# Deltares/pyflwdir

Hardware: AMD Instinct MI355X
Metric: Mcells/s upstream_area on D8 raster (higher is better)
Workload: dtype int32

## Files before the change

### pyflwdir_amd/csrc/tiled.h

```cpp
#pragma once
#include "common.h"

#define TS 64
#define TCELLS (TS * TS)
#define HW (TS + 2)
#define PSL 256
#define SG 8
#define SSL (SG * SG * PSL)
#define SSHIFT 14
#define SDONE 0x8000u
#define MAXROUNDS_SUPER 15
#define HG 4
#define HCAP 24576
#define HDONE 0x8000u
#define NPERIM (2 * TS + 2 * (TS - 2))
#define NONE32 0xFFFFFFFFu
#define PDONE 0x8000u
#define XDONE 0x80000000u
#define MAXROUNDS_TILE 13
#define CPT (TCELLS / 256)
#define ENC_SINK 0x80000000u
#define ENC_SIDE1 0x40000000u
#define ENC_COL 0x3FFFFFFFu

// ... 19 lines not shown
}
__host__ __device__ inline u32 xr_target12(u32 tr, u32 tc, u32 t12, u32 nstc);

__host__ __device__ inline u32 xr_target12(u32 tr, u32 tc, u32 t12, u32 nstc) {
  const u32 d = t12 >> 8;
  const u32 q = (d * 11u) >> 5;
  return sslot_base(tr + q - 1u, tc + (d - 3u * q) - 1u, nstc) + (t12 & 0xFFu);
}

__host__ __device__ inline u32 sb_index(u32 R, u32 C) {
  return R == 0u ? C : (R == SC - 1u ? SC + C : (C == 0u ? 2u * SC + (R - 1u) : 2u * SC + (SC - 2u) + (R - 1u)));
}
__host__ __device__ inline void sb_cell(u32 t, u32 *R, u32 *C) {
  if (t < SC) *R = 0u, *C = t;
  else if (t < 2u * SC) *R = SC - 1u, *C = t - SC;
  else if (t < 2u * SC + (SC - 2u)) *R = t - 2u * SC + 1u, *C = 0u;
  else *R = (t - (2u * SC + (SC - 2u)) + 1u) & (SC - 1u), *C = SC - 1u;
}

struct SuperArgs {
  u32 nst;
  const u32 *xT;
  const u32 *xrec;
  const u64 *xmask;
  uint16_t *xcb;
  uint16_t *xl_slot;
  uint16_t *xl_next;
  u32 *scount;
  u32 *nflag, *flagged;
  u32 *sb;
  uint16_t *R2L;
  u32 *sxidL;
  u32 *sx_slot;
  u32 *sx_n1;
  u32 *T3;
  u32 *xtot;
  u64 *ctrl;
  u32 nstc, nhtc;
  u32 *hcnt;
  int hmode;
  u32 edge_nstr;
  u32 ntr, ntc;
  u32 hcap;
  u8 *sover;
  u32 scap;
};

struct HyperArgs {
  const u32 *sx_slot;
  u32 *xtot;
  u32 nht;
  const u32 *hcnt;
  const u32 *T3;
  const u32 *J3;
  const u32 *xin3;
  u32 *T3out;
  u32 *R3;
  u32 *hx_id;
  u32 *hx_node;
  u32 *T4;
  u64 *ctrl;
  u32 edge_nstr, nhtc;
};

struct TileArgs {
  const u8 *ncode;
  const u8 *raw;
  u8 *ncode_w;
  u64 *tcnt;
  u64 ntot;
  u32 *hcnt;
  u32 nht;
  const i32 *weights;
  u32 nrow, ncol, ntr, ntc;
  u32 row_first, row_last;
  u32 nstc;
  u32 *xT;
  u32 *xrec;
  const u32 *xtot;
  u64 *xmask;
  u32 *esink;
  u32 *brow_first;
  u32 *haloA;
  u32 *brow_inflow;
  u64 *ctrl;
  i32 *out;
  u32 tr_lo, tr_hi, tc_lo, tc_hi;
  u64 *rcnt;
  u64 *stamps;
  int flags;
  const u64 *wrow = nullptr;
  const u32 *wfrac = nullptr;
  u64 *xT64 = nullptr;
};

__host__ __device__ inline u32 frame_tiles(u32 ntr, u32 ntc, u32 tr_lo, u32 tr_hi, u32 tc_lo, u32 tc_hi) {
  return ntr * ntc - (tr_hi - tr_lo) * (tc_hi - tc_lo);
}
__host__ __device__ inline void frame_tile(u32 id, u32 ntr, u32 ntc, u32 tr_lo, u32 tr_hi, u32 tc_lo, u32 tc_hi, u32 *tr,
                                           u32 *tc) {
  const u32 top = tr_lo * ntc, bot = (ntr - tr_hi) * ntc;
  if (id < top) {
    *tr = id / ntc, *tc = id % ntc;
  } else if (id < top + bot) {
    id -= top;
    *tr = tr_hi + id / ntc, *tc = id % ntc;
  } else {
    id -= top + bot;
    const u32 side = tc_lo + (ntc - tc_hi);
    const u32 x = id % side;
    *tr = tr_lo + id / side;
    *tc = x < tc_lo ? x : tc_hi + (x - tc_lo);
  }
}

// ... 65 lines not shown
    const i64 crr = gr < 0 ? 0 : (gr >= (i64)nrow ? (i64)nrow - 1 : gr);
    const i64 ccs = cs < 0 ? 0 : (cs >= (i64)ncol ? (i64)ncol - 1 : cs);
    u32 w;
    size_t off = (size_t)crr * ncol + (size_t)ccs;
    u32 sh = 0;
    if (GUARD && off + 4 > ntot) {
      sh = 8u * (u32)(off + 4 - ntot);
      off = ntot - 4;
    }
    __builtin_memcpy(&w, ncode + off, 4);
    if (GUARD) w >>= sh;
    const bool rowok = idx < HW * 18u && gr >= 0 && gr < (i64)nrow;
#pragma unroll
    for (int b = 0; b < 4; ++b) {
      const i64 col = cs + b;
      if (!rowok || col < 0 || col >= (i64)ncol) w = (w & ~(0xFFu << (8 * b))) | (D8_MV << (8 * b));
    }
    v[k] = w;
  }
}
__device__ __forceinline__ void stage_load_interior(const u8 *__restrict__ ncode, u32 ncol, i64 r0, i64 c0, u32 tid,
                                                    u32 (&v)[5]) {
  const u8 *base = ncode + (size_t)(r0 - 1) * ncol + (size_t)(c0 - 4);
#pragma unroll
  for (int k = 0; k < 5; ++k) {
    const u32 idx = tid + 256u * k;
    u32 hr = idx / 18u;
    const u32 d = idx - hr * 18u;
    hr = hr < HW - 1u ? hr : HW - 1u;
    __builtin_memcpy(&v[k], base + (size_t)hr * ncol + 4u * d, 4);
  }
}
__device__ __forceinline__ void stage_load_auto(const u8 *__restrict__ ncode, u32 nrow, u32 ncol, i64 r0, i64 c0, u32 tid,
                                                u32 (&v)[5]) {
  if (r0 >= 1 && c0 >= 4 && r0 + TS + 1 <= (i64)nrow && c0 + TS + 4 <= (i64)ncol) stage_load_interior(ncode, ncol, r0, c0, tid, v);
  else stage_load(ncode, nrow, ncol, r0, c0, tid, v);
}
__device__ __forceinline__ void stage_store(u8 *code, u32 tid, const u32 (&v)[5]) {
#pragma unroll
  for (int k = 0; k < 5; ++k) {
    const u32 idx = tid + 256u * k;
    if (idx < HW * 18u) ((u32 *)code)[idx] = v[k];
  }
}
#endif

struct TiledRun {
  pfd_raster *h = nullptr;
  u32 ntr = 0, ntc = 0, nexits = 0;
  size_t nslots = 0;
  bool supported = false, is_block = false, coarse_done = false, force_flat = false;
  DevBuf slots, sx, esink, bnd;
  u32 nst = 0, nstc = 0, nsuper = 0, nht = 0, nhtc = 0, nhyper = 0;
  DevBuf sbbuf, l3, l4, hcntbuf, tcntbuf, iface_buf, stampbuf, soverbuf, rcntbuf, xmaskbuf, xlbuf, scountbuf, flaggedbuf, xcbbuf;
  bool fused_norm = false;
  int rounds4 = 0, extra_rounds = 0;
  bool short_of_rounds = false;
  u32 *xT = nullptr, *xrec = nullptr, *xtot = nullptr, *sxidL = nullptr, *sx_slot = nullptr,
      *sx_n1 = nullptr;
  uint16_t *R2L = nullptr;
  SuperArgs sa{};
  u32 *brow_first = nullptr, *haloA = nullptr, *haloL = nullptr, *brow_sink = nullptr, *brow_inflow = nullptr;
  u32 *Tc = nullptr, *Tn = nullptr, *Jc = nullptr, *Jn = nullptr, *xin3 = nullptr, *R3 = nullptr, *hx_id = nullptr;
  size_t n3cap = 0, n4cap = 0;
  u32 *J4fin = nullptr;
  int solve_exits(const u32 *start, i64 *launches, bool cleared = false, bool edge_down = false);
  bool edge_down_now = false;
  int level3_flat(i64 *launches);
  int level3_flat_nosync(i64 *launches);
  bool flat_nosync = false;
  int level3_hyper(i64 *launches);
  int level4_down(i64 *launches);
  int resolve_with_inflow(i64 *launches);
  TileArgs a{};
  int init(pfd_raster *hh, i32 *out_dev);
  bool overflowed = false;
  int phase_a();
  int phase_a_checked();
  int phase_a_check();
  int phase_b(int *complete);
  int phase_b_issue();
  int phase_b_collect(const u64 *c0, int *complete);
  int stage_verdict_a();
  int block_verdict(int *flag_dev, bool host_ok);
  bool iface_doubling = false;
  u64 last_miss = 0;
  bool phase_a_needs_redo(const u64 *c8, int tries);
};

int pfd_doubling_rounds(pfd_raster *h, u32 *T[3], u32 *J[2], u32 n, int first_batch, bool check, bool *done,
                        int *rounds_issued, i64 *launches, const u64 *ncnt = nullptr, bool prepared = false);
```

### pyflwdir_amd/csrc/tiled.hip

```cpp
#include <stdio.h>
#include <stdlib.h>

#include <vector>

#include "common.h"
#include "tiled.h"

#define TSTAMP(slot)                                                                                        \
  if (a.flags & 16) {                                                                                       \
    __syncthreads();                                                                                        \
    if (tid == 0) {                                                                                         \
      const u64 t_ = __builtin_readcyclecounter();                                                          \
      atomicAdd((unsigned long long *)&a.stamps[(((tr * a.ntc + tc) & 1023u) << 3) + (FINAL ? 4 : 0) + slot], \
                (unsigned long long)(t_ - tprev));                                                        \
      tprev = t_;                                                                                           \
    }                                                                                                       \
  }

#define PREP 8
template <bool FINAL, bool RAW, bool INT, bool PERIM>
__device__ __forceinline__ void tile_body(const TileArgs &a, u32 *A, uint16_t *P, u8 *code, u64 *s_cnt, const u32 tr,
                                          const u32 tc) {
  u64 tprev = __builtin_readcyclecounter();
  const u32 tid = threadIdx.x;
// ... 686 lines not shown
      tot += c;
    }
    if (!tot) {
      s_base = 0;
    } else if (s.hmode) {
      const u32 b = atomicAdd(&s.hcnt[ht], tot);
      if (b + tot > s.hcap) s.ctrl[T_OVERFLOW] = 1;
      s_base = ht * HCAP + (b + tot > s.hcap ? 0u : b);
    } else {
      s_base = (u32)atomicAdd((unsigned long long *)&s.ctrl[T_NSUPER], (unsigned long long)tot);
    }
  }
  __syncthreads();
  u32 run = s_base + wtot[wave];
#pragma unroll
  for (int k = 0; k < DPT; ++k) {
    const u32 e = tid + NT * k;
    const bool sx = (sxbits >> k) & 1u;
    const u64 m = __ballot(sx);
    u32 id = NONE32;
    if (sx) {
      id = run + (u32)__popcll(m & ((1ull << lane) - 1ull));
      const u32 sl = (u32)s.xl_slot[base + e] & (SSL - 1);
      s.sx_slot[id] = base + sl;
      s.sx_n1[id] = xr_target12(str * SG + (sl >> 11), stc * SG + ((sl >> 8) & 7u), (u32)s.xl_next[base + e] & 0xFFFu, s.nstc);
      s.T3[id] = T[e];
    }
    run += (u32)__popcll(m);
    if (e < n) {
      s.R2L[base + e] = (uint16_t)(P[e] & (SDONE - 1u));
      s.sxidL[base + e] = id;
    }
  }
}

template <bool FINAL>
__global__ void __launch_bounds__(SNT, SNT == 512u ? 6 : 8) k_super(SuperArgs s) {
  if (s.sover[blockIdx.x]) return;
  super_solve<FINAL, SCAP, SNT>(s, blockIdx.x);
}
#define SFLAG_GRID 64u
template <bool FINAL>
__global__ void __launch_bounds__(1024, 4) k_super_flagged(SuperArgs s) {
  const u32 nf = *s.nflag;
  for (u32 f = blockIdx.x; f < nf; f += gridDim.x) {
    super_solve<FINAL, SSL, 1024u>(s, s.flagged[f]);
    __syncthreads();
  }
}

__device__ __forceinline__ bool sx_active(const SuperArgs &s, u32 k) {
  return !s.hmode || (k % HCAP) < s.hcnt[k / HCAP];
}
__global__ void __launch_bounds__(256) k_link3(SuperArgs s, u32 nsuper, u32 *__restrict__ J3,
                                               u32 *__restrict__ clear = nullptr) {
  const u32 k = blockIdx.x * blockDim.x + threadIdx.x;
  if (k >= nsuper) return;
  if (clear) clear[k] = 0;
  if (s.hmode && s.ctrl[T_OVERFLOW]) return;
  if (!sx_active(s, k)) {
    J3[k] = k | XDONE;
    return;
  }
  const u32 tgt = s.sx_n1[k];
  const u32 xe = (s.xrec[tgt] >> 8) & 0xFFu;
  u32 j = k | XDONE, pos = NONE32;
  if (xe != XR_NONE) {
    const u32 n1 = (tgt & ~255u) | xe, b1 = n1 & ~(u32)(SSL - 1);
    pos = b1 + xl_index(s.xmask, s.xcb, n1);
    const u32 id = s.sxidL[b1 + s.R2L[pos]];
    if (id != NONE32) j = id;
  }
  s.sx_n1[k] = pos;
  J3[k] = j;
}
__global__ void __launch_bounds__(256) k_sx_totals(SuperArgs s, u32 nsuper, const u32 *__restrict__ T3final) {
  const u32 k = blockIdx.x * blockDim.x + threadIdx.x;
  if (k < nsuper) s.xtot[s.sx_slot[k]] = T3final[k];
}

__global__ void __launch_bounds__(256) k_link3_flat(SuperArgs s, u32 cap, u32 *__restrict__ J3, u32 *__restrict__ Tnext) {
  const u32 n = min(cap, (u32)s.ctrl[T_NSUPER]);
  for (u32 k = blockIdx.x * blockDim.x + threadIdx.x; k < n; k += gridDim.x * blockDim.x) {
    Tnext[k] = 0;
    const u32 tgt = s.sx_n1[k];
    const u32 xe = (s.xrec[tgt] >> 8) & 0xFFu;
    u32 j = k | XDONE, pos = NONE32;
    if (xe != XR_NONE) {
      const u32 n1 = (tgt & ~255u) | xe, b1 = n1 & ~(u32)(SSL - 1);
      pos = b1 + xl_index(s.xmask, s.xcb, n1);
      const u32 id = s.sxidL[b1 + s.R2L[pos]];
      if (id != NONE32) j = id;
    }
    s.sx_n1[k] = pos;
    J3[k] = j;
  }
}
__global__ void __launch_bounds__(256) k_sx_totals_flat(SuperArgs s, u32 cap, const u32 *__restrict__ T3final) {
  const u32 n = min(cap, (u32)s.ctrl[T_NSUPER]);
  for (u32 k = blockIdx.x * blockDim.x + threadIdx.x; k < n; k += gridDim.x * blockDim.x) s.xtot[s.sx_slot[k]] = T3final[k];
}

template <bool FINAL>
__global__ void __launch_bounds__(1024) k_hyper(HyperArgs s) {
  __shared__ u32 T[HCAP];
  __shared__ uint16_t P[HCAP];
  __shared__ __attribute__((aligned(16))) u32 s_flag[2][16];
  __shared__ u32 s_cnt, s_base;
  const u32 tid = threadIdx.x;
  const u32 ht = blockIdx.x;
  const u32 base = ht * HCAP;
  if (s.ctrl[T_OVERFLOW]) return;
  if (FINAL && s.edge_nstr) {
    const u32 hr = ht / s.nhtc, n_ = s.edge_nstr;
    if (hr != 0 && hr < (n_ >= 3 ? (n_ - 3) / HG : 0u)) return;
  }
  const u32 n = s.hcnt[ht];
  constexpr int SPT = HCAP / 1024;
  if (tid == 0) s_cnt = 0;
  u32 y[SPT], ext = 0, live = 0;
#pragma unroll
  for (int j0 = 0; j0 < SPT; j0 += 8) {
    u32 j3s[8], ts[8];
    if (1024u * j0 < n) {
#pragma unroll
      for (int q = 0; q < 8; ++q) {
        const u32 i = tid + 1024u * (j0 + q);
        j3s[q] = s.J3[base + i];
        ts[q] = s.T3[base + i];
        if (FINAL) ts[q] += s.xin3[base + i];
      }
    }
#pragma unroll
    for (int q = 0; q < 8; ++q) {
      const int j = j0 + q;
      const u32 i = tid + 1024u * j;
      u32 p = i | HDONE, t = 0;
      if (i < n) {
        const u32 j3 = j3s[q];
        t = ts[q];
        if (!(j3 & XDONE)) {
          if (j3 / HCAP == ht)
            p = j3 % HCAP;
          else
            ext |= 1u << j;
        }
      }
      T[i] = t;
      P[i] = (uint16_t)p;
      y[j] = p & 0x7FFFu;
      if (!(p & HDONE)) live |= 1u << j;
    }
  }
  __syncthreads();
  for (int round = 0; round < 16; ++round) {
    u32 av[SPT], q[SPT];
#pragma unroll
    for (int j = 0; j < SPT; ++j) {
      if (live & (1u << j)) {
        av[j] = T[tid + 1024u * j];
        q[j] = P[y[j]];
      }
    }
    __syncthreads();
#pragma unroll
    for (int j = 0; j < SPT; ++j) {
      if (live & (1u << j)) {
        atomicAdd(&T[y[j]], av[j]);
        P[tid + 1024u * j] = (uint16_t)q[j];
        y[j] = q[j] & 0x7FFFu;
        if (q[j] & HDONE) live &= ~(1u << j);
      }
    }
    if (!wg_vote<16>(s_flag, round, tid, live != 0u)) break;
  }
  if (live) atomicAdd((unsigned long long *)&s.ctrl[T_SLIVE], 1ull);
  if (FINAL) {
#pragma unroll
    for (int j = 0; j < SPT; ++j) {
      const u32 i = tid + 1024u * j;
      if (i < n) {
        s.T3out[base + i] = T[i];
        s.xtot[s.sx_slot[base + i]] = T[i];
      }
    }
    return;
  }
  u32 rank[SPT];
#pragma unroll
  for (int j = 0; j < SPT; ++j) rank[j] = (ext & (1u << j)) ? atomicAdd(&s_cnt, 1u) : NONE32;
  __syncthreads();
  if (tid == 0) s_base = s_cnt ? (u32)atomicAdd((unsigned long long *)&s.ctrl[T_NHYPER], (unsigned long long)s_cnt) : 0u;
  __syncthreads();
#pragma unroll
  for (int j = 0; j < SPT; ++j) {
    const u32 i = tid + 1024u * j;
    if (i >= n) continue;
    s.T3out[base + i] = T[i];
    s.R3[base + i] = base + (P[i] & 0x7FFFu);
    u32 id = NONE32;
    if (rank[j] != NONE32) {
      id = s_base + rank[j];
      s.hx_node[id] = base + i;
      s.T4[id] = T[i];
    }
    s.hx_id[base + i] = id;
  }
}
__global__ void __launch_bounds__(256) k_link4(HyperArgs s, u32 cap, u32 *__restrict__ J4, u32 *__restrict__ Tnext) {
  if (s.ctrl[T_OVERFLOW]) return;
  const u32 n = min(cap, (u32)s.ctrl[T_NHYPER]);
  for (u32 m = blockIdx.x * blockDim.x + threadIdx.x; m < n; m += gridDim.x * blockDim.x) {
    Tnext[m] = 0;
    const u32 n1 = s.J3[s.hx_node[m]];
    const u32 id = s.hx_id[s.R3[n1]];
    const u32 j = (id != NONE32) ? id : (m | XDONE);
    J4[m] = j;
  }
}
__global__ void __launch_bounds__(256) k_push4(HyperArgs s, u32 cap, const u32 *__restrict__ T4final, u32 *xin3) {
  if (s.ctrl[T_OVERFLOW]) return;
  const u32 n = min(cap, (u32)s.ctrl[T_NHYPER]);
  for (u32 m = blockIdx.x * blockDim.x + threadIdx.x; m < n; m += gridDim.x * blockDim.x)
    atomicAdd(&xin3[s.J3[s.hx_node[m]]], T4final[m]);
}

__global__ void __launch_bounds__(256) k_coarse_round(const u32 *__restrict__ Told, u32 *__restrict__ Tnew,
                                                      u32 *__restrict__ Tzero, const u32 *__restrict__ Jold,
                                                      u32 *__restrict__ Jnew, u32 nexits, u64 *ctrl,
                                                      const u64 *__restrict__ ncnt, u32 round) {
  __shared__ u32 hk[512], hv[512];
  const u32 tid = threadIdx.x;
  if (ncnt) {
    nexits = ctrl[T_OVERFLOW] ? 0u : min(nexits, (u32)*ncnt);
  }
  bool moving = false;
  for (u32 base = blockIdx.x * blockDim.x; base < nexits; base += gridDim.x * blockDim.x) {
  hk[tid] = NONE32, hk[tid + 256u] = NONE32;
  hv[tid] = 0, hv[tid + 256u] = 0;
  const u32 e = base + tid;
  __syncthreads();
  if (e < nexits) {
    const u32 j = Jold[e];
    const u32 t = Told[e];
    Tzero[e] = 0;
    if (t) atomicAdd(&Tnew[e], t);
    if (j & XDONE) {
      Jnew[e] = j;
    } else {
      const u32 q = Jold[j];
      Jnew[e] = q;
      moving |= !(q & XDONE);
      if (t) {
        u32 slot = (j * 2654435761u) >> 23;
        for (;;) {
          const u32 prev = atomicCAS(&hk[slot], NONE32, j);
          if (prev == NONE32 || prev == j) {
            atomicAdd(&hv[slot], t);
            break;
          }
          slot = (slot + 1u) & 511u;
        }
      }
    }
  }
  __syncthreads();
#pragma unroll
  for (int k = 0; k < 2; ++k) {
    const u32 key = hk[tid + 256u * k], val = hv[tid + 256u * k];
    if (key != NONE32 && val) atomicAdd(&Tnew[key], val);
  }
  __syncthreads();
  }
  if (round && moving) {
    const u64 m = __ballot(1);
    if ((int)(threadIdx.x & 63) == __ffsll((long long)m) - 1) {
      if (__hip_atomic_load(&ctrl[T_XACTIVE], __ATOMIC_RELAXED, __HIP_MEMORY_SCOPE_AGENT) != (u64)round)
// ... 13 lines not shown
                        int *rounds_issued, i64 *launches, const u64 *ncnt, bool prepared) {
  const u32 grid = std::min(cdiv_u32(n, 256), 4096u);
  *done = false;
  if (!prepared) {
    HIPCHK(hipMemsetAsync(T[1], 0, (size_t)n * sizeof(u32), h->stream));
    HIPCHK(hipMemsetAsync(h->ctrl + T_XACTIVE, 0, sizeof(u64), h->stream));
  }
  int batch = first_batch, rounds = 0;
  while (rounds < 48 && !*done) {
    for (int b = 0; b < batch; ++b) {
      ++rounds;
      k_coarse_round<<<grid, 256, 0, h->stream>>>(T[0], T[1], T[2], J[0], J[1], n, h->ctrl, ncnt,
                                                  check ? (u32)rounds : 0u);
      ++*launches;
      u32 *t0 = T[0];
      T[0] = T[1], T[1] = T[2], T[2] = t0;
      std::swap(J[0], J[1]);
    }
    KCHK();
    if (!check) {
      k_check_saturated<<<grid, 256, 0, h->stream>>>(J[0], n, h->ctrl, ncnt, (u32)rounds);
      ++*launches;
      break;
    }
    u64 last = 0;
    HIPCHK(hipMemcpyAsync(&last, h->ctrl + T_XACTIVE, sizeof(u64), hipMemcpyDeviceToHost, h->stream));
    HIPCHK(hipStreamSynchronize(h->stream));
    *done = last < (u64)rounds;
    batch = 2;
  }
  *rounds_issued = rounds;
  return PFD_OK;
}

__global__ void __launch_bounds__(256) k_halo_collect(const u32 *__restrict__ esink, const u32 *__restrict__ xrec,
                                                      const u32 *__restrict__ xtot, u32 ntc, u32 ntr, u32 nstc, u32 ncol,
                                                      u32 *__restrict__ haloL, u32 n) {
  const u32 t = blockIdx.x * blockDim.x + threadIdx.x;
  if (t >= n) return;
  const u32 e = esink[t];
  if (e == NONE32) return;
  const u32 reg = t / (ntc * PSL), tc = (t % (ntc * PSL)) / PSL, p = t % PSL;
  const u32 tr = reg ? ntr - 1 : 0;
  int lr, lc;
  pslot_inv((int)p, &lr, &lc);
  const u32 v = slot_inflow(xtot, xrec[sslot_base(tr, tc, nstc) + p], tr, tc, lr, lc, nstc);
  if (v) atomicAdd(&haloL[((e & ENC_SIDE1) ? ncol : 0u) + (e & ENC_COL)], v);
}
struct LastExitArgs {
  const u64 *xmask;
  const uint16_t *xcb, *xl_slot, *R2L;
  const u32 *sxidL, *sx_slot, *sx_n1, *xrec;
  const u32 *J3;
  const u32 *R3, *hx_id, *hx_node, *J4fin;
  int hmode;
};
__device__ __forceinline__ u32 last_exit(const LastExitArgs &q, u32 f) {
  const u32 b = f & ~(u32)(SSL - 1);
  const u32 r2 = q.R2L[b + xl_index(q.xmask, q.xcb, f)];
  const u32 k = q.sxidL[b + r2];
  if (k == NONE32) return b + (q.xl_slot[b + r2] & (SSL - 1));
  u32 k3;
  if (q.hmode) {
    k3 = q.R3[k];
    const u32 m = q.hx_id[k3];
    if (m != NONE32) {
      const u32 mlast = q.J4fin[m] & ~XDONE;
      k3 = q.R3[q.J3[q.hx_node[mlast]] & ~XDONE];
    }
  } else {
    k3 = q.J3[k] & ~XDONE;
  }
  const u32 pos = q.sx_n1[k3];
  if (pos == NONE32) return q.sx_slot[k3];
  const u32 b2 = pos & ~(u32)(SSL - 1);
  return b2 + (q.xl_slot[b2 + q.R2L[pos]] & (SSL - 1));
}
__global__ void __launch_bounds__(256) k_brow_sink(const u32 *__restrict__ brow_first, LastExitArgs q,
                                                   const u32 *__restrict__ esink, u32 ntc, u32 ntr, u32 nstc, u32 ncol,
                                                   u32 *__restrict__ brow_sink, const u64 *__restrict__ ctrl) {
  const u32 t = blockIdx.x * blockDim.x + threadIdx.x;
  if (t >= 2 * ncol) return;
  if (q.hmode && ctrl[T_OVERFLOW]) return;
  u32 f = brow_first[t];
  if (f != NONE32 && !(f & ENC_SINK)) {
    const u32 le = last_exit(q, f);
    u32 tr, tc, p;
    sslot_inv(xr_target(le, q.xrec[le], nstc), nstc, &tr, &tc, &p);
    f = NONE32;
    if (tr == 0)
      f = esink[(size_t)tc * PSL + p];
    else if (tr == ntr - 1)
      f = esink[((size_t)ntc + tc) * PSL + p];
  }
  brow_sink[t] = f;
}
__global__ void __launch_bounds__(256) k_brow_scatter(const u32 *__restrict__ brow_first, const u32 *__restrict__ brow_inflow,
                                                      u32 ncol, u32 *__restrict__ start) {
  const u32 t = blockIdx.x * blockDim.x + threadIdx.x;
  if (t >= 2 * ncol) return;
  const u32 v = brow_inflow[t], e = brow_first[t];
  if (v && e != NONE32 && !(e & ENC_SINK)) atomicAdd(&start[e], v);
}

__global__ void __launch_bounds__(256) k_brow_scatter_delta(const u32 *__restrict__ brow_first, const u32 *__restrict__ brow_inflow,
                                                            u32 ncol, u32 *__restrict__ start, const u64 *__restrict__ xmask,
                                                            const uint16_t *__restrict__ xcb, const uint16_t *__restrict__ R2L,
                                                            const u32 *__restrict__ sxidL, u32 *__restrict__ T3,
                                                            const u32 *__restrict__ R3, const u32 *__restrict__ hx_id,
                                                            u32 *__restrict__ T4start, const u64 *__restrict__ ctrl) {
  const u32 t = blockIdx.x * blockDim.x + threadIdx.x;
  if (t >= 2 * ncol) return;
  if (ctrl[T_OVERFLOW]) return;
  const u32 v = brow_inflow[t], e = brow_first[t];
  if (!v || e == NONE32 || (e & ENC_SINK)) return;
  atomicAdd(&start[e], v);
  const u32 b = e & ~(u32)(SSL - 1);
  const u32 id = sxidL[b + R2L[b + xl_index(xmask, xcb, e)]];
  if (id == NONE32) return;
  atomicAdd(&T3[id], v);
  const u32 m = hx_id[R3[id]];
  if (m != NONE32) atomicAdd(&T4start[m], v);
}
__global__ void __launch_bounds__(256) k_l4_restart(const u32 *__restrict__ T4saved, u32 *__restrict__ T4, u32 n4, u32 *__restrict__ xin3,
                                                    u32 n3, u64 *__restrict__ ctrl) {
  const u32 i0 = blockIdx.x * blockDim.x + threadIdx.x, stride = gridDim.x * blockDim.x;
  for (u32 i = i0; i < n4; i += stride) T4[i] = T4saved[i];
  for (u32 i = i0; i < n3; i += stride) xin3[i] = 0;
  if (i0 == 0) ctrl[T_XACTIVE] = 0;
}
__global__ void __launch_bounds__(256) k_pass_clear(u64 *__restrict__ ctrl, u32 ctrl_from, u32 *__restrict__ bnd, u32 nb,
                                                    uint4 *__restrict__ xmask16, u32 n16) {
  const u32 i0 = blockIdx.x * blockDim.x + threadIdx.x, stride = gridDim.x * blockDim.x;
  if (i0 < 64u && i0 >= ctrl_from) ctrl[i0] = 0;
  for (u32 i = i0; i < 5u * nb; i += stride) {
    const u32 reg = i / nb;
    bnd[i] = (reg == 0u || reg == 3u) ? NONE32 : 0u;
  }
  for (u32 i = i0; i < n16; i += stride) xmask16[i] = make_uint4(0u, 0u, 0u, 0u);
}
__global__ void k_stage_verdict_a(u64 *ctrl, u32 hmode, u32 rounds4) {
  u64 m = 0;
  if (ctrl[T_OVERFLOW]) m |= MISS_OVERFLOW;
  if (hmode && rounds4 && ctrl[T_XACTIVE] >= (u64)rounds4) m |= MISS_ROUNDS4;
  if (m) ctrl[T_MISS] |= m;
}
__global__ void k_block_verdict(const u64 *ctrl, u32 hmode, u32 rounds4, u32 host_ok, int *flag) {
  const bool redo = ctrl[T_OVERFLOW] != 0 || ctrl[T_MISS] != 0 || (hmode && rounds4 && ctrl[T_XACTIVE] >= (u64)rounds4);
  const bool fine = host_ok && ctrl[T_SLIVE] == 0 && ctrl[T_UNSAT] == 0 && ctrl[2] == 0;
  *flag = redo ? 1 : (fine ? 2 : 0);
}

int TiledRun::init(pfd_raster *hh, i32 *out_dev) {
  h = hh;
  ntr = cdiv_u32((u64)h->nrow, TS);
  ntc = cdiv_u32((u64)h->ncol, TS);
  nstc = cdiv_u32(ntc, SG);
  const u32 nstr = cdiv_u32(ntr, SG);
  nst = nstr * nstc;
  nhtc = cdiv_u32(nstc, HG);
  nht = cdiv_u32(nstr, HG) * nhtc;
  nslots = (size_t)nst * SSL;
  supported = !(nslots >= 0x3FFFFFFFull || ntr > 65535u || (u64)h->ncol >= ENC_SIDE1 ||
                (size_t)nht * HCAP >= 0x7FFFFFFFull);
  if (!supported) return PFD_OK;
  const size_t nb = 2 * (size_t)h->ncol;
  const size_t sxcap = (size_t)nst * 4 * SG * TS;
  n3cap = std::max(sxcap, (size_t)nht * HCAP);
  n4cap = (size_t)nht * 4 * HG * SG * TS;
  PFDCHK(slots.alloc(4 * nslots * sizeof(u32) + nslots * sizeof(uint16_t)));
  PFDCHK(sbbuf.alloc((size_t)nst * SBN * sizeof(u32)));
  PFDCHK(l3.alloc(9 * n3cap * sizeof(u32)));
  PFDCHK(l4.alloc(7 * n4cap * sizeof(u32)));
  PFDCHK(hcntbuf.alloc((size_t)nht * sizeof(u32)));
  PFDCHK(esink.alloc(2 * (size_t)ntc * PSL * sizeof(u32)));
  PFDCHK(bnd.alloc(5 * nb * sizeof(u32)));
  u32 *q = slots.as<u32>();
  xT = q, xrec = q + nslots, xtot = q + 2 * nslots, sxidL = q + 3 * nslots;
  R2L = (uint16_t *)(q + 4 * nslots);
  u32 *x = l3.as<u32>();
  sx_slot = x;
  Tc = x + n3cap, Tn = x + 2 * n3cap, Jc = x + 3 * n3cap, Jn = x + 4 * n3cap;
  xin3 = x + 5 * n3cap, R3 = x + 6 * n3cap, hx_id = x + 7 * n3cap;
  sx_n1 = x + 8 * n3cap;
  u32 *b = bnd.as<u32>();
  brow_first = b;
  haloA = b + nb;
  haloL = b + 2 * nb;
  brow_sink = b + 3 * nb;
  brow_inflow = b + 4 * nb;
  a = TileArgs{h->ncode, nullptr, h->ncode, nullptr, (u64)h->n, hcntbuf.as<u32>(), nht, nullptr, (u32)h->nrow, (u32)h->ncol, ntr, ntc, (u32)h->halo_top,
               (u32)(h->halo_top + h->own_rows - 1), nstc, xT, xrec, xtot, nullptr, esink.as<u32>(),
               brow_first, haloA, brow_inflow, h->ctrl, out_dev, 0};
  sa = SuperArgs{};
  sa.nst = nst, sa.xT = xT, sa.xrec = xrec, sa.sb = sbbuf.as<u32>(), sa.R2L = R2L, sa.sxidL = sxidL, sa.sx_slot = sx_slot,
  sa.sx_n1 = sx_n1, sa.T3 = Tc, sa.xtot = xtot, sa.ctrl = h->ctrl, sa.nstc = nstc, sa.nhtc = nhtc,
  sa.hcnt = hcntbuf.as<u32>(), sa.ntr = ntr, sa.ntc = ntc, sa.hcap = HCAP, sa.scap = SCAP;
  PFDCHK(soverbuf.alloc((size_t)nst));
  sa.sover = soverbuf.as<u8>();
  PFDCHK(xmaskbuf.alloc(nslots / 64 * sizeof(u64) + 8 + 16));
  PFDCHK(xlbuf.alloc(2 * nslots * sizeof(uint16_t)));
  PFDCHK(scountbuf.alloc((size_t)nst * sizeof(u32)));
  PFDCHK(xcbbuf.alloc(nslots / 64 * sizeof(uint16_t)));
  sa.xcb = xcbbuf.as<uint16_t>();
  a.xmask = xmaskbuf.as<u64>();
  sa.xmask = xmaskbuf.as<u64>();
  sa.xl_slot = xlbuf.as<uint16_t>();
  sa.xl_next = xlbuf.as<uint16_t>() + nslots;
  sa.scount = scountbuf.as<u32>();
  sa.nflag = (u32 *)(xmaskbuf.as<u64>() + nslots / 64);
  PFDCHK(flaggedbuf.alloc((size_t)nst * sizeof(u32)));
  sa.flagged = flaggedbuf.as<u32>();
  if (const char *e = pfd_knob("PFD_TEST_HCAP")) sa.hcap = (u32)std::min(atoi(e), HCAP);
  if (const char *e = pfd_knob("PFD_TEST_SCAP")) sa.scap = (u32)std::min<u32>((u32)atoi(e), SCAP);
  a.stamps = nullptr;
#ifdef PFD_DEVTOOLS
  if (const char *e = getenv("PFD_TILE_ABLATE")) a.flags = atoi(e) & 16;
  if (a.flags & 16) {
    PFDCHK(stampbuf.alloc(8192 * sizeof(u64)));
    a.stamps = stampbuf.as<u64>();
    HIPCHK(hipMemsetAsync(a.stamps, 0, 8192 * sizeof(u64), h->stream));
  }
#endif
  if (h->count_rounds) {
    a.flags |= 32;
    PFDCHK(rcntbuf.alloc(1024 * sizeof(u64)));
    HIPCHK(hipMemsetAsync(rcntbuf.p, 0, 1024 * sizeof(u64), h->stream));
    a.rcnt = rcntbuf.as<u64>();
  }
  is_block = h->halo_top || h->halo_bot;
  a.tr_lo = (a.row_first + 1u + TS - 1u) / TS;
  a.tr_hi = a.row_last >= TS ? a.row_last / TS : 0u;
  a.tc_lo = 1u;
  a.tc_hi = a.ncol >= TS + 4u ? (a.ncol - 4u) / TS : 0u;
  if (a.tr_hi <= a.tr_lo || a.tc_hi <= a.tc_lo || pfd_knob("PFD_TILE_GENERAL")) a.tr_lo = a.tr_hi = a.tc_lo = a.tc_hi = 0u;
  return PFD_OK;
}

int TiledRun::level3_flat(i64 *launches) {
  const u32 g3 = cdiv_u32(nsuper, 256);
  k_link3<<<g3, 256, 0, h->stream>>>(sa, nsuper, Jc);
  ++*launches;
  int batch = 1;
  for (u32 span = 1; span < (ntr + ntc) / SG + 2; span <<= 1) ++batch;
  bool done3 = false;
  u32 *T[3] = {Tc, Tn, xin3}, *J[2] = {Jc, Jn};
  int rounds = 0;
  PFDCHK(pfd_doubling_rounds(h, T, J, nsuper, batch + 2, true, &done3, &rounds, launches, nullptr));
  Tc = T[0], Tn = T[1], Jc = J[0], Jn = J[1];
  coarse_done = coarse_done && done3;
  k_sx_totals<<<g3, 256, 0, h->stream>>>(sa, nsuper, Tc);
  ++*launches;
  KCHK();
  return PFD_OK;
}

#define FLAT_MAX_HT 64u
int TiledRun::level3_flat_nosync(i64 *launches) {
  const u32 cap3 = (u32)std::min<size_t>(n3cap, 0x7FFFFFFF);
  const u32 g3 = std::min(cdiv_u32(cap3, 256), 4096u);
  k_link3_flat<<<g3, 256, 0, h->stream>>>(sa, cap3, Jc, Tn);
  int batch = 7 + extra_rounds;
  for (u32 span = 1; span < (ntr + ntc) / SG + 2; span <<= 1) ++batch;
  if (const char *e = pfd_knob("PFD_TEST_ROUNDS4")) batch = atoi(e) + extra_rounds;
  bool done3 = false;
  u32 *T[3] = {Tc, Tn, xin3}, *J[2] = {Jc, Jn};
  PFDCHK(pfd_doubling_rounds(h, T, J, cap3, batch, false, &done3, &rounds4, launches, h->ctrl + T_NSUPER, true));
  Tc = T[0], Tn = T[1], xin3 = T[2], Jc = J[0], Jn = J[1];
  k_sx_totals_flat<<<g3, 256, 0, h->stream>>>(sa, cap3, Tc);
  *launches += 2;
  KCHK();
  return PFD_OK;
}

int TiledRun::level3_hyper(i64 *launches) {
  const u32 n3 = nht * HCAP;
  const u32 g3 = cdiv_u32(n3, 256);
  u32 *T3 = Tc, *J3 = Jc, *T3out = Tn;
  u32 *y = l4.as<u32>();
  u32 *hx_node = y, *T4c = y + n4cap;
  k_link3<<<g3, 256, 0, h->stream>>>(sa, n3, J3, xin3);
  HyperArgs ha{sx_slot, xtot, nht, hcntbuf.as<u32>(), T3, J3, xin3, T3out, R3, hx_id, hx_node, T4c, h->ctrl,
               edge_down_now ? cdiv_u32(ntr, SG) : 0u, nhtc};
  k_hyper<false><<<nht, 1024, 0, h->stream>>>(ha);
  KCHK();
  *launches += 2;
  if (is_block)
    HIPCHK(hipMemcpyAsync(y + 6 * n4cap, T4c, n4cap * sizeof(u32), hipMemcpyDeviceToDevice, h->stream));
  return level4_down(launches);
}

int TiledRun::level4_down(i64 *launches) {
  u32 *T3 = Tc, *J3 = Jc, *T3out = Tn;
  u32 *y = l4.as<u32>();
  u32 *hx_node = y, *T4c = y + n4cap, *J4c = y + 3 * n4cap;
  u32 *T4[3] = {y + n4cap, y + 2 * n4cap, y + 5 * n4cap}, *J4[2] = {y + 3 * n4cap, y + 4 * n4cap};
  HyperArgs ha{sx_slot, xtot, nht, hcntbuf.as<u32>(), T3, J3, xin3, T3out, R3, hx_id, hx_node, T4c, h->ctrl,
               edge_down_now ? cdiv_u32(ntr, SG) : 0u, nhtc};
  {
    const u32 cap4 = (u32)std::min<size_t>(n4cap, 0x7FFFFFFF);
    const u32 g4 = std::min(cdiv_u32(cap4, 256), 4096u);
    k_link4<<<g4, 256, 0, h->stream>>>(ha, cap4, J4c, T4[1]);
    int batch = 5 + extra_rounds;
    for (u32 span = 1; span < (ntr + ntc) / (SG * HG) + 2; span <<= 1) ++batch;
    if (const char *e = pfd_knob("PFD_TEST_ROUNDS4")) batch = atoi(e) + extra_rounds;
    bool done4 = false;
    PFDCHK(pfd_doubling_rounds(h, T4, J4, cap4, batch, false, &done4, &rounds4, launches, h->ctrl + T_NHYPER, true));
    J4fin = J4[0];
    k_push4<<<g4, 256, 0, h->stream>>>(ha, cap4, T4[0], xin3);
    *launches += 2;
  }
  k_hyper<true><<<nht, 1024, 0, h->stream>>>(ha);
  *launches += 1;
  KCHK();
  return PFD_OK;
}

int TiledRun::resolve_with_inflow(i64 *launches) {
  edge_down_now = false;
  sa.edge_nstr = 0;
  sa.xT = xT;
  const size_t nb = 2 * (size_t)h->ncol;
  u32 *y = l4.as<u32>();
  k_brow_scatter_delta<<<cdiv_u32(nb, 256), 256, 0, h->stream>>>(brow_first, brow_inflow, (u32)h->ncol, xT, sa.xmask, sa.xcb, R2L,
                                                                sxidL, Tc, R3, hx_id, y + 6 * n4cap, h->ctrl);
  const u32 n3 = (u32)((size_t)nht * HCAP), n4 = (u32)n4cap;
  k_l4_restart<<<std::min(cdiv_u32(std::max(n3, n4), 256), 2048u), 256, 0, h->stream>>>(y + 6 * n4cap, y + n4cap, n4, xin3, n3, h->ctrl);
  *launches += 2;
  PFDCHK(level4_down(launches));
  k_super<true><<<nst, SNT, 0, h->stream>>>(sa);
  k_super_flagged<true><<<std::min<u32>(nst, SFLAG_GRID), 1024, 0, h->stream>>>(sa);
  *launches += 2;
  KCHK();
  return PFD_OK;
}

int TiledRun::solve_exits(const u32 *start, i64 *launches, bool cleared, bool edge_down) {
  edge_down_now = edge_down;
  sa.edge_nstr = edge_down ? cdiv_u32(ntr, SG) : 0u;
  if (!cleared) {
    HIPCHK(hipMemsetAsync(hcntbuf.p, 0, (size_t)nht * sizeof(u32), h->stream));
    HIPCHK(hipMemsetAsync(h->ctrl + T_XACTIVE, 0, 3 * sizeof(u64), h->stream));
  }
  sa.xT = start;
  Tc = l3.as<u32>() + n3cap, Tn = Tc + n3cap, Jc = Tn + n3cap, Jn = Jc + n3cap;
  sa.T3 = Tc;
  sa.hmode = (nht > 1 && !force_flat && !pfd_knob("PFD_FLAT_L3")) ? 1 : 0;
  const char *hs = pfd_knob("PFD_HYPER_SMALL");
  flat_nosync = !is_block && sa.hmode && nht <= FLAT_MAX_HT && !(hs && atoi(hs) != 0);
  if (flat_nosync) sa.hmode = 0;
  xin3 = l3.as<u32>() + 5 * n3cap;
  k_super<false><<<nst, SNT, 0, h->stream>>>(sa);
  k_super_flagged<false><<<std::min<u32>(nst, SFLAG_GRID), 1024, 0, h->stream>>>(sa);
  KCHK();
  *launches += 2;
  if (flat_nosync) {
    PFDCHK(level3_flat_nosync(launches));
  } else if (!sa.hmode) {
    u64 c[8];
    HIPCHK(hipMemcpyAsync(c, h->ctrl + 8, sizeof(c), hipMemcpyDeviceToHost, h->stream));
    HIPCHK(hipStreamSynchronize(h->stream));
    nsuper = (u32)c[T_NSUPER - 8];
  }
  if (flat_nosync) {
  } else if (sa.hmode)
    PFDCHK(level3_hyper(launches));
  else if (nsuper)
    PFDCHK(level3_flat(launches));
  k_super<true><<<nst, SNT, 0, h->stream>>>(sa);
  k_super_flagged<true><<<std::min<u32>(nst, SFLAG_GRID), 1024, 0, h->stream>>>(sa);
  *launches += 2;
  KCHK();
  return PFD_OK;
}

int TiledRun::phase_a() {
  coarse_done = true;
  const size_t nb = 2 * (size_t)h->ncol;
  {
    const size_t xbytes = nslots / 64 * sizeof(u64) + 8;
    const u32 n16 = (u32)((xbytes + 15) / 16);
    const u32 work = std::max<u32>(n16, is_block ? (u32)(5 * nb) : 0u);
    k_pass_clear<<<std::max(1u, std::min(cdiv_u32(work, 256), 4096u)), 256, 0, h->stream>>>(
        h->ctrl, h->normalised ? 8u : 0u, bnd.as<u32>(), is_block ? (u32)nb : 0u, (uint4 *)a.xmask, n16);
  }
  const dim3 gridi(a.tc_hi - a.tc_lo, a.tr_hi - a.tr_lo);
  const bool have_i = gridi.x && gridi.y;
  const u32 gridf = frame_tiles(ntr, ntc, a.tr_lo, a.tr_hi, a.tc_lo, a.tc_hi);
  pfd_seg_begin(h, "tile_local");
  if (!h->normalised) {
    if (!tcntbuf.p) PFDCHK(tcntbuf.alloc((size_t)ntr * ntc * sizeof(u64)));
    a.raw = h->raw;
    a.tcnt = tcntbuf.as<u64>();
    if (have_i) {
      if (a.weights) k_tile_local_fast<true, true><<<gridi, 256, 0, h->stream>>>(a);
      else if (a.xT64) k_tile_local_fast<true, false, true><<<gridi, 256, 0, h->stream>>>(a);
      else k_tile_local_fast<true, false><<<gridi, 256, 0, h->stream>>>(a);
      pfd_seg_end(h, 1);
      pfd_seg_begin(h, "tile_local_frame");
    }
    if (is_block)
      k_tile<false, true><<<gridf, 256, 0, h->stream>>>(a);
    else
      k_tile<false, true, true><<<gridf, 256, 0, h->stream>>>(a);
// ... 172 lines not shown
```

Baseline: 213,500.

## Fuse level-3 linking and level-4 push into hyper-tile kernels via neighbor-bucketed exits

Folds the k_link3 pass into k_hyper<false>, which now computes J3 links inline. Exits are bucketed by which of the 8 neighbouring hyper-tiles they target, with per-tile offsets stored in a new hxoff buffer. k_hyper<true> then gathers incoming level-4 totals from its neighbours' buckets and adds them with shared-memory atomics. This replaces the k_push4 global atomic scatter into xin3 and the zeroing of xin3 on restart. Two launches and a global atomic array go away, in exchange for more register pressure and prologue work in k_hyper, and an assumption that hyper exits only reach adjacent hyper-tiles.

```diff
diff --git a/pyflwdir_amd/csrc/tiled.h b/pyflwdir_amd/csrc/tiled.h
--- a/pyflwdir_amd/csrc/tiled.h
+++ b/pyflwdir_amd/csrc/tiled.h
@@ -95,15 +95,20 @@
   u32 nht;
   const u32 *hcnt;
   const u32 *T3;
-  const u32 *J3;
-  const u32 *xin3;
+  u32 *J3;
   u32 *T3out;
   u32 *R3;
   u32 *hx_id;
-  u32 *hx_node;
+  u32 *hx_tgt;
+  u32 *hxoff;
+  const u32 *T4fin;
   u32 *T4;
   u64 *ctrl;
   u32 edge_nstr, nhtc;
+  u32 *sx_n1;
+  const u32 *xrec, *sxidL;
+  const u64 *xmask;
+  const uint16_t *xcb, *R2L;
 };
 
 struct TileArgs {
@@ -275,7 +280,8 @@
   bool supported = false, is_block = false, coarse_done = false, force_flat = false;
   DevBuf slots, sx, esink, bnd;
   u32 nst = 0, nstc = 0, nsuper = 0, nht = 0, nhtc = 0, nhyper = 0;
-  DevBuf sbbuf, l3, l4, hcntbuf, tcntbuf, iface_buf, stampbuf, soverbuf, rcntbuf, xmaskbuf, xlbuf, scountbuf, flaggedbuf, xcbbuf;
+  DevBuf sbbuf, l3, l4, hcntbuf, tcntbuf, iface_buf, stampbuf, soverbuf, rcntbuf, xmaskbuf, xlbuf, scountbuf, flaggedbuf, xcbbuf,
+      hxoffbuf;
   bool fused_norm = false;
   int rounds4 = 0, extra_rounds = 0;
   bool short_of_rounds = false;
@@ -284,7 +290,8 @@
   uint16_t *R2L = nullptr;
   SuperArgs sa{};
   u32 *brow_first = nullptr, *haloA = nullptr, *haloL = nullptr, *brow_sink = nullptr, *brow_inflow = nullptr;
-  u32 *Tc = nullptr, *Tn = nullptr, *Jc = nullptr, *Jn = nullptr, *xin3 = nullptr, *R3 = nullptr, *hx_id = nullptr;
+  u32 *Tc = nullptr, *Tn = nullptr, *Jc = nullptr, *Jn = nullptr, *Tz = nullptr, *R3 = nullptr, *hx_id = nullptr;
+  HyperArgs hyper_args(u32 *T4fin);
   size_t n3cap = 0, n4cap = 0;
   u32 *J4fin = nullptr;
   int solve_exits(const u32 *start, i64 *launches, bool cleared = false, bool edge_down = false);
diff --git a/pyflwdir_amd/csrc/tiled.hip b/pyflwdir_amd/csrc/tiled.hip
--- a/pyflwdir_amd/csrc/tiled.hip
+++ b/pyflwdir_amd/csrc/tiled.hip
@@ -762,16 +762,9 @@
 __device__ __forceinline__ bool sx_active(const SuperArgs &s, u32 k) {
   return !s.hmode || (k % HCAP) < s.hcnt[k / HCAP];
 }
-__global__ void __launch_bounds__(256) k_link3(SuperArgs s, u32 nsuper, u32 *__restrict__ J3,
-                                               u32 *__restrict__ clear = nullptr) {
+__global__ void __launch_bounds__(256) k_link3(SuperArgs s, u32 nsuper, u32 *__restrict__ J3) {
   const u32 k = blockIdx.x * blockDim.x + threadIdx.x;
   if (k >= nsuper) return;
-  if (clear) clear[k] = 0;
-  if (s.hmode && s.ctrl[T_OVERFLOW]) return;
-  if (!sx_active(s, k)) {
-    J3[k] = k | XDONE;
-    return;
-  }
   const u32 tgt = s.sx_n1[k];
   const u32 xe = (s.xrec[tgt] >> 8) & 0xFFu;
   u32 j = k | XDONE, pos = NONE32;
@@ -816,7 +809,7 @@
   __shared__ u32 T[HCAP];
   __shared__ uint16_t P[HCAP];
   __shared__ __attribute__((aligned(16))) u32 s_flag[2][16];
-  __shared__ u32 s_cnt, s_base;
+  __shared__ u32 s_cnt[9], s_off[10];
   const u32 tid = threadIdx.x;
   const u32 ht = blockIdx.x;
   const u32 base = ht * HCAP;
@@ -825,20 +818,77 @@
     const u32 hr = ht / s.nhtc, n_ = s.edge_nstr;
     if (hr != 0 && hr < (n_ >= 3 ? (n_ - 3) / HG : 0u)) return;
   }
+  const u32 hr = ht / s.nhtc, hc = ht % s.nhtc;
+  constexpr int PU = 4;
+  u32 blo[8], bcum[9], pt[PU], pv[PU];
+  auto hx_at = [&](u32 x) -> u32 {
+    u32 m = 0;
+#pragma unroll
+    for (int g = 0; g < 8; ++g) m = x >= bcum[g] ? blo[g] + (x - bcum[g]) : m;
+    return m;
+  };
+  if (FINAL) {
+    const u32 nhtr = s.nht / s.nhtc;
+    bcum[0] = 0;
+#pragma unroll
+    for (int g = 0; g < 8; ++g) {
+      const u32 d = (u32)g + (g >= 4 ? 1u : 0u);
+      const u32 ar = hr + d / 3u - 1u, ac = hc + d % 3u - 1u;
+      const bool ok = ar < nhtr && ac < s.nhtc;
+      const u32 a = ok ? ar * s.nhtc + ac : 0u;
+      const u32 lo = s.hxoff[a * 10u + 8u - d], hi = s.hxoff[a * 10u + 9u - d];
+      blo[g] = lo;
+      bcum[g + 1] = bcum[g] + (ok ? hi - lo : 0u);
+    }
+#pragma unroll
+    for (int u = 0; u < PU; ++u) {
+      const u32 x = tid + 1024u * u;
+      const u32 m = x < bcum[8] ? hx_at(x) : 0u;
+      pt[u] = s.hx_tgt[m];
+      pv[u] = s.T4fin[m];
+    }
+  }
   const u32 n = s.hcnt[ht];
   constexpr int SPT = HCAP / 1024;
-  if (tid == 0) s_cnt = 0;
+  if (!FINAL && tid < 9u) s_cnt[tid] = 0;
   u32 y[SPT], ext = 0, live = 0;
+  u32 hd[SPT / 8] = {};
 #pragma unroll
   for (int j0 = 0; j0 < SPT; j0 += 8) {
     u32 j3s[8], ts[8];
     if (1024u * j0 < n) {
+      u32 tg[8];
 #pragma unroll
       for (int q = 0; q < 8; ++q) {
         const u32 i = tid + 1024u * (j0 + q);
-        j3s[q] = s.J3[base + i];
         ts[q] = s.T3[base + i];
-        if (FINAL) ts[q] += s.xin3[base + i];
+        if (FINAL) j3s[q] = s.J3[base + i];
+        else tg[q] = s.sx_n1[base + i];
+      }
+      if (!FINAL) {
+        u32 xe[8], pos[8];
+#pragma unroll
+        for (int q = 0; q < 8; ++q) {
+          tg[q] = tid + 1024u * (j0 + q) < n ? tg[q] : 0u;
+          xe[q] = (s.xrec[tg[q]] >> 8) & 0xFFu;
+        }
+#pragma unroll
+        for (int q = 0; q < 8; ++q) {
+          const u32 n1 = (tg[q] & ~255u) | xe[q];
+          const u32 li = (u32)s.xcb[n1 >> 6] + (u32)__popcll(s.xmask[n1 >> 6] & ((1ull << (n1 & 63u)) - 1ull));
+          pos[q] = (n1 & ~(u32)(SSL - 1)) + (li & (SSL - 1));
+        }
+#pragma unroll
+        for (int q = 0; q < 8; ++q) {
+          const u32 i = tid + 1024u * (j0 + q);
+          const u32 id = s.sxidL[(pos[q] & ~(u32)(SSL - 1)) + ((u32)s.R2L[pos[q]] & (SSL - 1))];
+          const bool ok = xe[q] != XR_NONE;
+          j3s[q] = ok && id != NONE32 ? id : (base + i) | XDONE;
+          if (i < n) {
+            s.sx_n1[base + i] = ok ? pos[q] : NONE32;
+            s.J3[base + i] = j3s[q];
+          }
+        }
       }
     }
 #pragma unroll
@@ -850,10 +900,16 @@
         const u32 j3 = j3s[q];
         t = ts[q];
         if (!(j3 & XDONE)) {
-          if (j3 / HCAP == ht)
+          const u32 th = j3 / HCAP;
+          if (th == ht) {
             p = j3 % HCAP;
-          else
+          } else {
             ext |= 1u << j;
+            if (!FINAL) {
+              const u32 d = 3u * (th / s.nhtc + 1u - hr) + (th % s.nhtc + 1u - hc);
+              hd[j >> 3] |= d << (4 * (j & 7));
+            }
+          }
         }
       }
       T[i] = t;
@@ -863,6 +919,18 @@
     }
   }
   __syncthreads();
+  if (FINAL) {
+#pragma unroll
+    for (int u = 0; u < PU; ++u) {
+      const u32 l = pt[u] - base;
+      if (tid + 1024u * u < bcum[8] && l < HCAP) atomicAdd(&T[l], pv[u]);
+    }
+    for (u32 x = tid + 1024u * PU; x < bcum[8]; x += 1024u) {
+      const u32 m = hx_at(x), l = s.hx_tgt[m] - base;
+      if (l < HCAP) atomicAdd(&T[l], s.T4fin[m]);
+    }
+    __syncthreads();
+  }
   for (int round = 0; round < 16; ++round) {
     u32 av[SPT], q[SPT];
 #pragma unroll
@@ -898,10 +966,24 @@
   }
   u32 rank[SPT];
 #pragma unroll
-  for (int j = 0; j < SPT; ++j) rank[j] = (ext & (1u << j)) ? atomicAdd(&s_cnt, 1u) : NONE32;
+  for (int j = 0; j < SPT; ++j) {
+    const u32 d = (hd[j >> 3] >> (4 * (j & 7))) & 15u;
+    rank[j] = (ext & (1u << j)) ? atomicAdd(&s_cnt[d], 1u) | (d << 16) : NONE32;
+  }
   __syncthreads();
-  if (tid == 0) s_base = s_cnt ? (u32)atomicAdd((unsigned long long *)&s.ctrl[T_NHYPER], (unsigned long long)s_cnt) : 0u;
+  if (tid == 0) {
+    u32 tot = 0;
+    for (int d = 0; d < 9; ++d) {
+      const u32 c = s_cnt[d];
+      s_off[d] = tot;
+      tot += c;
+    }
+    const u32 b = tot ? (u32)atomicAdd((unsigned long long *)&s.ctrl[T_NHYPER], (unsigned long long)tot) : 0u;
+    for (int d = 0; d < 9; ++d) s_off[d] += b;
+    s_off[9] = b + tot;
+  }
   __syncthreads();
+  if (tid < 10u) s.hxoff[ht * 10u + tid] = s_off[tid];
 #pragma unroll
   for (int j = 0; j < SPT; ++j) {
     const u32 i = tid + 1024u * j;
@@ -910,8 +992,8 @@
     s.R3[base + i] = base + (P[i] & 0x7FFFu);
     u32 id = NONE32;
     if (rank[j] != NONE32) {
-      id = s_base + rank[j];
-      s.hx_node[id] = base + i;
+      id = s_off[rank[j] >> 16] + (rank[j] & 0xFFFFu);
+      s.hx_tgt[id] = s.J3[base + i];
       s.T4[id] = T[i];
     }
     s.hx_id[base + i] = id;
@@ -922,17 +1004,10 @@
   const u32 n = min(cap, (u32)s.ctrl[T_NHYPER]);
   for (u32 m = blockIdx.x * blockDim.x + threadIdx.x; m < n; m += gridDim.x * blockDim.x) {
     Tnext[m] = 0;
-    const u32 n1 = s.J3[s.hx_node[m]];
-    const u32 id = s.hx_id[s.R3[n1]];
+    const u32 id = s.hx_id[s.R3[s.hx_tgt[m]]];
     const u32 j = (id != NONE32) ? id : (m | XDONE);
     J4[m] = j;
   }
-}
-__global__ void __launch_bounds__(256) k_push4(HyperArgs s, u32 cap, const u32 *__restrict__ T4final, u32 *xin3) {
-  if (s.ctrl[T_OVERFLOW]) return;
-  const u32 n = min(cap, (u32)s.ctrl[T_NHYPER]);
-  for (u32 m = blockIdx.x * blockDim.x + threadIdx.x; m < n; m += gridDim.x * blockDim.x)
-    atomicAdd(&xin3[s.J3[s.hx_node[m]]], T4final[m]);
 }
 
 __global__ void __launch_bounds__(256) k_coarse_round(const u32 *__restrict__ Told, u32 *__restrict__ Tnew,
@@ -1052,7 +1127,7 @@
   const uint16_t *xcb, *xl_slot, *R2L;
   const u32 *sxidL, *sx_slot, *sx_n1, *xrec;
   const u32 *J3;
-  const u32 *R3, *hx_id, *hx_node, *J4fin;
+  const u32 *R3, *hx_id, *hx_tgt, *J4fin;
   int hmode;
 };
 __device__ __forceinline__ u32 last_exit(const LastExitArgs &q, u32 f) {
@@ -1066,7 +1141,7 @@
     const u32 m = q.hx_id[k3];
     if (m != NONE32) {
       const u32 mlast = q.J4fin[m] & ~XDONE;
-      k3 = q.R3[q.J3[q.hx_node[mlast]] & ~XDONE];
+      k3 = q.R3[q.hx_tgt[mlast]];
     }
   } else {
     k3 = q.J3[k] & ~XDONE;
@@ -1122,11 +1197,10 @@
   const u32 m = hx_id[R3[id]];
   if (m != NONE32) atomicAdd(&T4start[m], v);
 }
-__global__ void __launch_bounds__(256) k_l4_restart(const u32 *__restrict__ T4saved, u32 *__restrict__ T4, u32 n4, u32 *__restrict__ xin3,
-                                                    u32 n3, u64 *__restrict__ ctrl) {
+__global__ void __launch_bounds__(256) k_l4_restart(const u32 *__restrict__ T4saved, u32 *__restrict__ T4, u32 n4,
+                                                    u64 *__restrict__ ctrl) {
   const u32 i0 = blockIdx.x * blockDim.x + threadIdx.x, stride = gridDim.x * blockDim.x;
   for (u32 i = i0; i < n4; i += stride) T4[i] = T4saved[i];
-  for (u32 i = i0; i < n3; i += stride) xin3[i] = 0;
   if (i0 == 0) ctrl[T_XACTIVE] = 0;
 }
 __global__ void __launch_bounds__(256) k_pass_clear(u64 *__restrict__ ctrl, u32 ctrl_from, u32 *__restrict__ bnd, u32 nb,
@@ -1173,6 +1247,7 @@
   PFDCHK(l3.alloc(9 * n3cap * sizeof(u32)));
   PFDCHK(l4.alloc(7 * n4cap * sizeof(u32)));
   PFDCHK(hcntbuf.alloc((size_t)nht * sizeof(u32)));
+  PFDCHK(hxoffbuf.alloc((size_t)nht * 10 * sizeof(u32)));
   PFDCHK(esink.alloc(2 * (size_t)ntc * PSL * sizeof(u32)));
   PFDCHK(bnd.alloc(5 * nb * sizeof(u32)));
   u32 *q = slots.as<u32>();
@@ -1181,7 +1256,7 @@
   u32 *x = l3.as<u32>();
   sx_slot = x;
   Tc = x + n3cap, Tn = x + 2 * n3cap, Jc = x + 3 * n3cap, Jn = x + 4 * n3cap;
-  xin3 = x + 5 * n3cap, R3 = x + 6 * n3cap, hx_id = x + 7 * n3cap;
+  Tz = x + 5 * n3cap, R3 = x + 6 * n3cap, hx_id = x + 7 * n3cap;
   sx_n1 = x + 8 * n3cap;
   u32 *b = bnd.as<u32>();
   brow_first = b;
@@ -1244,7 +1319,7 @@
   int batch = 1;
   for (u32 span = 1; span < (ntr + ntc) / SG + 2; span <<= 1) ++batch;
   bool done3 = false;
-  u32 *T[3] = {Tc, Tn, xin3}, *J[2] = {Jc, Jn};
+  u32 *T[3] = {Tc, Tn, Tz}, *J[2] = {Jc, Jn};
   int rounds = 0;
   PFDCHK(pfd_doubling_rounds(h, T, J, nsuper, batch + 2, true, &done3, &rounds, launches, nullptr));
   Tc = T[0], Tn = T[1], Jc = J[0], Jn = J[1];
@@ -1264,39 +1339,40 @@
   for (u32 span = 1; span < (ntr + ntc) / SG + 2; span <<= 1) ++batch;
   if (const char *e = pfd_knob("PFD_TEST_ROUNDS4")) batch = atoi(e) + extra_rounds;
   bool done3 = false;
-  u32 *T[3] = {Tc, Tn, xin3}, *J[2] = {Jc, Jn};
+  u32 *T[3] = {Tc, Tn, Tz}, *J[2] = {Jc, Jn};
   PFDCHK(pfd_doubling_rounds(h, T, J, cap3, batch, false, &done3, &rounds4, launches, h->ctrl + T_NSUPER, true));
-  Tc = T[0], Tn = T[1], xin3 = T[2], Jc = J[0], Jn = J[1];
+  Tc = T[0], Tn = T[1], Tz = T[2], Jc = J[0], Jn = J[1];
   k_sx_totals_flat<<<g3, 256, 0, h->stream>>>(sa, cap3, Tc);
   *launches += 2;
   KCHK();
   return PFD_OK;
 }
 
+HyperArgs TiledRun::hyper_args(u32 *T4fin) {
+  u32 *y = l4.as<u32>();
+  HyperArgs ha{};
+  ha.sx_slot = sx_slot, ha.xtot = xtot, ha.nht = nht, ha.hcnt = hcntbuf.as<u32>(), ha.T3 = Tc, ha.J3 = Jc, ha.T3out = Tn;
+  ha.R3 = R3, ha.hx_id = hx_id, ha.hx_tgt = y, ha.hxoff = hxoffbuf.as<u32>(), ha.T4fin = T4fin, ha.T4 = y + n4cap;
+  ha.ctrl = h->ctrl, ha.edge_nstr = edge_down_now ? cdiv_u32(ntr, SG) : 0u, ha.nhtc = nhtc;
+  ha.sx_n1 = sx_n1, ha.xrec = xrec, ha.sxidL = sxidL, ha.xmask = sa.xmask, ha.xcb = sa.xcb, ha.R2L = R2L;
+  return ha;
+}
+
 int TiledRun::level3_hyper(i64 *launches) {
-  const u32 n3 = nht * HCAP;
-  const u32 g3 = cdiv_u32(n3, 256);
-  u32 *T3 = Tc, *J3 = Jc, *T3out = Tn;
   u32 *y = l4.as<u32>();
-  u32 *hx_node = y, *T4c = y + n4cap;
-  k_link3<<<g3, 256, 0, h->stream>>>(sa, n3, J3, xin3);
-  HyperArgs ha{sx_slot, xtot, nht, hcntbuf.as<u32>(), T3, J3, xin3, T3out, R3, hx_id, hx_node, T4c, h->ctrl,
-               edge_down_now ? cdiv_u32(ntr, SG) : 0u, nhtc};
-  k_hyper<false><<<nht, 1024, 0, h->stream>>>(ha);
+  k_hyper<false><<<nht, 1024, 0, h->stream>>>(hyper_args(nullptr));
   KCHK();
-  *launches += 2;
+  *launches += 1;
   if (is_block)
-    HIPCHK(hipMemcpyAsync(y + 6 * n4cap, T4c, n4cap * sizeof(u32), hipMemcpyDeviceToDevice, h->stream));
+    HIPCHK(hipMemcpyAsync(y + 6 * n4cap, y + n4cap, n4cap * sizeof(u32), hipMemcpyDeviceToDevice, h->stream));
   return level4_down(launches);
 }
 
 int TiledRun::level4_down(i64 *launches) {
-  u32 *T3 = Tc, *J3 = Jc, *T3out = Tn;
   u32 *y = l4.as<u32>();
-  u32 *hx_node = y, *T4c = y + n4cap, *J4c = y + 3 * n4cap;
+  u32 *J4c = y + 3 * n4cap;
   u32 *T4[3] = {y + n4cap, y + 2 * n4cap, y + 5 * n4cap}, *J4[2] = {y + 3 * n4cap, y + 4 * n4cap};
-  HyperArgs ha{sx_slot, xtot, nht, hcntbuf.as<u32>(), T3, J3, xin3, T3out, R3, hx_id, hx_node, T4c, h->ctrl,
-               edge_down_now ? cdiv_u32(ntr, SG) : 0u, nhtc};
+  const HyperArgs ha = hyper_args(nullptr);
   {
     const u32 cap4 = (u32)std::min<size_t>(n4cap, 0x7FFFFFFF);
     const u32 g4 = std::min(cdiv_u32(cap4, 256), 4096u);
@@ -1307,11 +1383,10 @@
     bool done4 = false;
     PFDCHK(pfd_doubling_rounds(h, T4, J4, cap4, batch, false, &done4, &rounds4, launches, h->ctrl + T_NHYPER, true));
     J4fin = J4[0];
-    k_push4<<<g4, 256, 0, h->stream>>>(ha, cap4, T4[0], xin3);
-    *launches += 2;
-  }
-  k_hyper<true><<<nht, 1024, 0, h->stream>>>(ha);
-  *launches += 1;
+    *launches += 1;
+    k_hyper<true><<<nht, 1024, 0, h->stream>>>(hyper_args(T4[0]));
+    *launches += 1;
+  }
   KCHK();
   return PFD_OK;
 }
@@ -1324,8 +1399,8 @@
   u32 *y = l4.as<u32>();
   k_brow_scatter_delta<<<cdiv_u32(nb, 256), 256, 0, h->stream>>>(brow_first, brow_inflow, (u32)h->ncol, xT, sa.xmask, sa.xcb, R2L,
                                                                 sxidL, Tc, R3, hx_id, y + 6 * n4cap, h->ctrl);
-  const u32 n3 = (u32)((size_t)nht * HCAP), n4 = (u32)n4cap;
-  k_l4_restart<<<std::min(cdiv_u32(std::max(n3, n4), 256), 2048u), 256, 0, h->stream>>>(y + 6 * n4cap, y + n4cap, n4, xin3, n3, h->ctrl);
+  const u32 n4 = (u32)n4cap;
+  k_l4_restart<<<std::min(cdiv_u32(n4, 256), 2048u), 256, 0, h->stream>>>(y + 6 * n4cap, y + n4cap, n4, h->ctrl);
   *launches += 2;
   PFDCHK(level4_down(launches));
   k_super<true><<<nst, SNT, 0, h->stream>>>(sa);
@@ -1349,7 +1424,7 @@
   const char *hs = pfd_knob("PFD_HYPER_SMALL");
   flat_nosync = !is_block && sa.hmode && nht <= FLAT_MAX_HT && !(hs && atoi(hs) != 0);
   if (flat_nosync) sa.hmode = 0;
-  xin3 = l3.as<u32>() + 5 * n3cap;
+  Tz = l3.as<u32>() + 5 * n3cap;
   k_super<false><<<nst, SNT, 0, h->stream>>>(sa);
   k_super_flagged<false><<<std::min<u32>(nst, SFLAG_GRID), 1024, 0, h->stream>>>(sa);
   KCHK();
```

Result: faster. 215,800, median of 6 (+1.1%).
